# phoreproject/prysm

Measured on AMD Instinct MI355X. Metric: tree-hash leaves/sec @2^28 chunks (ssz.merkleHash, 32-B leaves), higher is better.
Workload: dtype u64 (Keccak lanes as u32 pairs)

## Files before the change

### prysm_amd/csrc/keccak_dev.hpp

```cpp
#pragma once
#include <hip/hip_runtime.h>
#include <stdint.h>

#include "plan_types.hpp"

namespace mk {

__constant__ uint32_t kRcLo[24] = {
    0x00000001u, 0x00008082u, 0x0000808Au, 0x80008000u, 0x0000808Bu, 0x80000001u,
    0x80008081u, 0x00008009u, 0x0000008Au, 0x00000088u, 0x80008009u, 0x8000000Au,
    0x8000808Bu, 0x0000008Bu, 0x00008089u, 0x00008003u, 0x00008002u, 0x00000080u,
    0x0000800Au, 0x8000000Au, 0x80008081u, 0x00008080u, 0x80000001u, 0x80008008u};
__constant__ uint32_t kRcHi[24] = {
    0x00000000u, 0x00000000u, 0x80000000u, 0x80000000u, 0x00000000u, 0x00000000u,
    0x80000000u, 0x80000000u, 0x00000000u, 0x00000000u, 0x00000000u, 0x00000000u,
    0x00000000u, 0x80000000u, 0x80000000u, 0x80000000u, 0x80000000u, 0x80000000u,
    0x00000000u, 0x80000000u, 0x80000000u, 0x80000000u, 0x00000000u, 0x80000000u};

__device__ __forceinline__ uint32_t xor3(uint32_t a, uint32_t b, uint32_t c) {
    return __builtin_amdgcn_bitop3_b32(a, b, c, 0x96);
}
__device__ __forceinline__ uint32_t chi3(uint32_t a, uint32_t b, uint32_t c) {
    return __builtin_amdgcn_bitop3_b32(a, b, c, 0xD2);
}
__device__ __forceinline__ uint32_t funnel(uint32_t hi, uint32_t lo, uint32_t s) {
    return __builtin_amdgcn_alignbit(hi, lo, s);
}

template <int N>
__device__ __forceinline__ void rotl64(uint32_t lo, uint32_t hi, uint32_t& olo, uint32_t& ohi) {
    if constexpr (N == 0) {
        olo = lo;
        ohi = hi;
    } else if constexpr (N == 32) {
        olo = hi;
        ohi = lo;
    } else if constexpr (N < 32) {
        ohi = funnel(hi, lo, 32 - N);
        olo = funnel(lo, hi, 32 - N);
    } else {
        ohi = funnel(lo, hi, 64 - N);
        olo = funnel(hi, lo, 64 - N);
    }
}

struct State {
    uint32_t lo[25];
    uint32_t hi[25];
};

__device__ __forceinline__ void zero(State& s) {
#pragma unroll
    for (int i = 0; i < 25; ++i) {
        s.lo[i] = 0u;
        s.hi[i] = 0u;
    }
}

#define MK_RHO(i)                                                                          \
    ((i) == 0 ? 0 : (i) == 1 ? 1 : (i) == 2 ? 62 : (i) == 3 ? 28 : (i) == 4 ? 27          \
   : (i) == 5 ? 36 : (i) == 6 ? 44 : (i) == 7 ? 6 : (i) == 8 ? 55 : (i) == 9 ? 20          \
   : (i) == 10 ? 3 : (i) == 11 ? 10 : (i) == 12 ? 43 : (i) == 13 ? 25 : (i) == 14 ? 39    \
   : (i) == 15 ? 41 : (i) == 16 ? 45 : (i) == 17 ? 15 : (i) == 18 ? 21 : (i) == 19 ? 8    \
   : (i) == 20 ? 18 : (i) == 21 ? 2 : (i) == 22 ? 61 : (i) == 23 ? 56 : 14)

template <int I>
__device__ __forceinline__ void rho_pi_one(const State& a, uint32_t (&blo)[25], uint32_t (&bhi)[25]) {
    constexpr int x = I % 5, y = I / 5;
    constexpr int dst = y + 5 * ((2 * x + 3 * y) % 5);
    rotl64<MK_RHO(I)>(a.lo[I], a.hi[I], blo[dst], bhi[dst]);
}

template <int... Is>
__device__ __forceinline__ void rho_pi_all(const State& a, uint32_t (&blo)[25], uint32_t (&bhi)[25],
                                           std::integer_sequence<int, Is...>) {
    (rho_pi_one<Is>(a, blo, bhi), ...);
}

__device__ __forceinline__ uint32_t ax3(uint32_t a, uint32_t b, uint32_t c) {
    uint32_t r;
    asm volatile("v_bitop3_b32 %0, %1, %2, %3 bitop3:0x96" : "=v"(r) : "v"(a), "v"(b), "v"(c));
    return r;
}
__device__ __forceinline__ uint32_t achi(uint32_t a, uint32_t b, uint32_t c) {
    uint32_t r;
    asm volatile("v_bitop3_b32 %0, %1, %2, %3 bitop3:0xd2" : "=v"(r) : "v"(a), "v"(b), "v"(c));
    return r;
}
template <int S>
__device__ __forceinline__ uint32_t aalign(uint32_t hi, uint32_t lo) {
    uint32_t r;
    asm volatile("v_alignbit_b32 %0, %1, %2, %3" : "=v"(r) : "v"(hi), "v"(lo), "i"(S));
    return r;
}
__device__ __forceinline__ uint32_t axs(uint32_t a, uint32_t s) {
    uint32_t r;
    asm volatile("v_xor_b32 %0, %1, %2" : "=v"(r) : "s"(s), "v"(a));
    return r;
}
template <int N>
__device__ __forceinline__ void arot(uint32_t lo, uint32_t hi, uint32_t& olo, uint32_t& ohi) {
    if constexpr (N == 0) {
        olo = lo;
        ohi = hi;
    } else if constexpr (N < 32) {
        ohi = aalign<32 - N>(hi, lo);
        olo = aalign<32 - N>(lo, hi);
    } else {
        ohi = aalign<64 - N>(lo, hi);
        olo = aalign<64 - N>(hi, lo);
    }
}
template <int I>
__device__ __forceinline__ void arho(const State& a, uint32_t (&blo)[25], uint32_t (&bhi)[25]) {
    constexpr int x = I % 5, y = I / 5;
    constexpr int dst = y + 5 * ((2 * x + 3 * y) % 5);
    arot<MK_RHO(I)>(a.lo[I], a.hi[I], blo[dst], bhi[dst]);
}
template <int... Is>
__device__ __forceinline__ void arho_all(const State& a, uint32_t (&blo)[25], uint32_t (&bhi)[25],
                                         std::integer_sequence<int, Is...>) {
    (arho<Is>(a, blo, bhi), ...);
}

template <bool BAR = false>
__device__ __forceinline__ void round_asm(State& s, uint32_t rclo, uint32_t rchi) {
    uint32_t clo[5], chi_[5];
#pragma unroll
    for (int x = 0; x < 5; ++x) {
        clo[x] = ax3(s.lo[x], s.lo[x + 5], s.lo[x + 10]);
        chi_[x] = ax3(s.hi[x], s.hi[x + 5], s.hi[x + 10]);
    }
#pragma unroll
    for (int x = 0; x < 5; ++x) {
        clo[x] = ax3(clo[x], s.lo[x + 15], s.lo[x + 20]);
        chi_[x] = ax3(chi_[x], s.hi[x + 15], s.hi[x + 20]);
    }
    uint32_t rlo[5], rhi[5];
#pragma unroll
    for (int x = 0; x < 5; ++x) arot<1>(clo[x], chi_[x], rlo[x], rhi[x]);
    if constexpr (BAR && MK_LOCK_BARS >= 2) __builtin_amdgcn_s_barrier();
#pragma unroll
    for (int i = 0; i < 25; ++i) {
        const int x = i % 5;
        s.lo[i] = ax3(s.lo[i], clo[(x + 4) % 5], rlo[(x + 1) % 5]);
        s.hi[i] = ax3(s.hi[i], chi_[(x + 4) % 5], rhi[(x + 1) % 5]);
    }
    uint32_t blo[25], bhi[25];
    arho_all(s, blo, bhi, std::make_integer_sequence<int, 25>{});
    if constexpr (BAR) __builtin_amdgcn_s_barrier();
#pragma unroll
    for (int y = 0; y < 5; ++y) {
#pragma unroll
        for (int x = 0; x < 5; ++x) {
            const int i = x + 5 * y;
            const int i1 = (x + 1) % 5 + 5 * y, i2 = (x + 2) % 5 + 5 * y;
            s.lo[i] = achi(blo[i], blo[i1], blo[i2]);
            s.hi[i] = achi(bhi[i], bhi[i1], bhi[i2]);
        }
    }
    s.lo[0] = axs(s.lo[0], rclo);
    s.hi[0] = axs(s.hi[0], rchi);
}

__device__ __forceinline__ void round_fn(State& s, uint32_t rclo, uint32_t rchi) { round_asm(s, rclo, rchi); }

#ifndef MK_ROUND_UNROLL
#define MK_ROUND_UNROLL 2
#endif
constexpr int kRoundUnroll = MK_ROUND_UNROLL;

__device__ __forceinline__ void keccak_f(State& s) {
#pragma unroll kRoundUnroll
    for (int r = 0; r < 24; ++r) round_fn(s, kRcLo[r], kRcHi[r]);
}

template <int X>
__device__ __forceinline__ void diag_rho(const State& s, const uint32_t (&clo)[5], const uint32_t (&chi_)[5],
                                         const uint32_t (&rlo)[5], const uint32_t (&rhi)[5], uint32_t (&blo)[5],
                                         uint32_t (&bhi)[5]) {
    constexpr int i = 6 * X;
    const uint32_t alo = xor3(s.lo[i], clo[(X + 4) % 5], rlo[(X + 1) % 5]);
    const uint32_t ahi = xor3(s.hi[i], chi_[(X + 4) % 5], rhi[(X + 1) % 5]);
    rotl64<MK_RHO(i)>(alo, ahi, blo[X], bhi[X]);
}

__device__ __forceinline__ void last_round_digest(State& s, uint32_t rclo, uint32_t rchi) {
    uint32_t clo[5], chi_[5];
#pragma unroll
    for (int x = 0; x < 5; ++x) {
        clo[x] = xor3(xor3(s.lo[x], s.lo[x + 5], s.lo[x + 10]), s.lo[x + 15], s.lo[x + 20]);
        chi_[x] = xor3(xor3(s.hi[x], s.hi[x + 5], s.hi[x + 10]), s.hi[x + 15], s.hi[x + 20]);
    }
    uint32_t rlo[5], rhi[5];
#pragma unroll
    for (int x = 0; x < 5; ++x) rotl64<1>(clo[x], chi_[x], rlo[x], rhi[x]);
    uint32_t blo[5], bhi[5];
    diag_rho<0>(s, clo, chi_, rlo, rhi, blo, bhi);
    diag_rho<1>(s, clo, chi_, rlo, rhi, blo, bhi);
    diag_rho<2>(s, clo, chi_, rlo, rhi, blo, bhi);
    diag_rho<3>(s, clo, chi_, rlo, rhi, blo, bhi);
    diag_rho<4>(s, clo, chi_, rlo, rhi, blo, bhi);
#pragma unroll
    for (int x = 0; x < 4; ++x) {
        s.lo[x] = chi3(blo[x], blo[(x + 1) % 5], blo[(x + 2) % 5]);
        s.hi[x] = chi3(bhi[x], bhi[(x + 1) % 5], bhi[(x + 2) % 5]);
    }
    s.lo[0] ^= rclo;
    s.hi[0] ^= rchi;
}

__device__ __forceinline__ void keccak_f_digest(State& s) {
#pragma unroll kRoundUnroll
    for (int r = 0; r < 22; ++r) round_fn(s, kRcLo[r], kRcHi[r]);
    round_fn(s, kRcLo[22], kRcHi[22]);
    last_round_digest(s, kRcLo[23], kRcHi[23]);
    asm volatile("" : "+v"(s.lo[0]), "+v"(s.hi[0]), "+v"(s.lo[1]), "+v"(s.hi[1]), "+v"(s.lo[2]), "+v"(s.hi[2]),
                 "+v"(s.lo[3]), "+v"(s.hi[3]));
}

__device__ __forceinline__ void keccak_f_lock(State& s) {
#pragma unroll kRoundUnroll
    for (int r = 0; r < 24; ++r) round_asm<true>(s, kRcLo[r], kRcHi[r]);
}
template <int K, typename F>
__device__ __forceinline__ void keccak_f_lock_mid(State& s, F&& mid) {
    static_assert(K >= 0 && K <= 24, "mid point");
    if constexpr (K == 0) mid();
#pragma unroll kRoundUnroll
    for (int r = 0; r < K; ++r) round_asm<true>(s, kRcLo[r], kRcHi[r]);
    if constexpr (K > 0) mid();
#pragma unroll kRoundUnroll
    for (int r = K; r < 24; ++r) round_asm<true>(s, kRcLo[r], kRcHi[r]);
}
template <int K1, int K2, typename F1, typename F2>
__device__ __forceinline__ void keccak_f_lock_mid2(State& s, F1&& m1, F2&& m2) {
    static_assert(K1 > 0 && K1 < K2 && K2 < 24, "mid points");
#pragma unroll kRoundUnroll
    for (int r = 0; r < K1; ++r) round_asm<true>(s, kRcLo[r], kRcHi[r]);
    m1();
#pragma unroll kRoundUnroll
    for (int r = K1; r < K2; ++r) round_asm<true>(s, kRcLo[r], kRcHi[r]);
    m2();
#pragma unroll kRoundUnroll
    for (int r = K2; r < 24; ++r) round_asm<true>(s, kRcLo[r], kRcHi[r]);
}
template <int K1, int K2, int K3, typename F1, typename F2, typename F3>
__device__ __forceinline__ void keccak_f_lock_mid3(State& s, F1&& m1, F2&& m2, F3&& m3) {
    static_assert(K1 > 0 && K1 < K2 && K2 < K3 && K3 < 24, "mid points");
#pragma unroll kRoundUnroll
    for (int r = 0; r < K1; ++r) round_asm<true>(s, kRcLo[r], kRcHi[r]);
    m1();
#pragma unroll kRoundUnroll
    for (int r = K1; r < K2; ++r) round_asm<true>(s, kRcLo[r], kRcHi[r]);
    m2();
#pragma unroll kRoundUnroll
    for (int r = K2; r < K3; ++r) round_asm<true>(s, kRcLo[r], kRcHi[r]);
    m3();
#pragma unroll kRoundUnroll
    for (int r = K3; r < 24; ++r) round_asm<true>(s, kRcLo[r], kRcHi[r]);
}
template <int K = 0, typename F>
__device__ __forceinline__ void keccak_f_digest_lock(State& s, F&& mid) {
    static_assert(K >= 0 && K <= 22, "mid point");
    if constexpr (K == 0) mid();
#pragma unroll kRoundUnroll
    for (int r = 0; r < K; ++r) round_asm<true>(s, kRcLo[r], kRcHi[r]);
    if constexpr (K > 0) mid();
#pragma unroll kRoundUnroll
    for (int r = K; r < 22; ++r) round_asm<true>(s, kRcLo[r], kRcHi[r]);
    round_asm<true>(s, kRcLo[22], kRcHi[22]);
    last_round_digest(s, kRcLo[23], kRcHi[23]);
    asm volatile("" : "+v"(s.lo[0]), "+v"(s.hi[0]), "+v"(s.lo[1]), "+v"(s.hi[1]), "+v"(s.lo[2]), "+v"(s.hi[2]),
                 "+v"(s.lo[3]), "+v"(s.hi[3]));
}
template <int K1, int K2, int K3, typename F1, typename F2, typename F3>
__device__ __forceinline__ void keccak_f_digest_lock_mid3(State& s, F1&& m1, F2&& m2, F3&& m3) {
    static_assert(K1 > 0 && K1 < K2 && K2 < K3 && K3 <= 22, "mid points");
#pragma unroll kRoundUnroll
    for (int r = 0; r < K1; ++r) round_asm<true>(s, kRcLo[r], kRcHi[r]);
    m1();
#pragma unroll kRoundUnroll
    for (int r = K1; r < K2; ++r) round_asm<true>(s, kRcLo[r], kRcHi[r]);
    m2();
#pragma unroll kRoundUnroll
    for (int r = K2; r < K3; ++r) round_asm<true>(s, kRcLo[r], kRcHi[r]);
    m3();
#pragma unroll kRoundUnroll
    for (int r = K3; r < 22; ++r) round_asm<true>(s, kRcLo[r], kRcHi[r]);
    round_asm<true>(s, kRcLo[22], kRcHi[22]);
    last_round_digest(s, kRcLo[23], kRcHi[23]);
    asm volatile("" : "+v"(s.lo[0]), "+v"(s.hi[0]), "+v"(s.lo[1]), "+v"(s.hi[1]), "+v"(s.lo[2]), "+v"(s.hi[2]),
                 "+v"(s.lo[3]), "+v"(s.hi[3]));
}
__device__ __forceinline__ void keccak_f_digest_lock(State& s) {
#pragma unroll kRoundUnroll
    for (int r = 0; r < 22; ++r) round_asm<true>(s, kRcLo[r], kRcHi[r]);
    round_asm<true>(s, kRcLo[22], kRcHi[22]);
    last_round_digest(s, kRcLo[23], kRcHi[23]);
    asm volatile("" : "+v"(s.lo[0]), "+v"(s.hi[0]), "+v"(s.lo[1]), "+v"(s.hi[1]), "+v"(s.lo[2]), "+v"(s.hi[2]),
                 "+v"(s.lo[3]), "+v"(s.hi[3]));
}

__device__ __forceinline__ void xor_lane(State& s, int i, uint2 w) {
    s.lo[i] ^= w.x;
    s.hi[i] ^= w.y;
}

template <int POS>
__device__ __forceinline__ void pad_const(State& s) {
    constexpr int lane = POS / 8, sh = (POS % 8) * 8;
    if constexpr (sh < 32)
        s.lo[lane] ^= 1u << sh;
    else
        s.hi[lane] ^= 1u << (sh - 32);
    s.hi[16] ^= 0x80000000u;
}

typedef unsigned int u32x4_t __attribute__((ext_vector_type(4)));
typedef unsigned int u32x2_t __attribute__((ext_vector_type(2)));
__device__ __forceinline__ uint4 ld_stream(const uint4* p) { return *p; }
__device__ __forceinline__ uint2 ld_stream(const uint2* p) { return *p; }

__device__ __forceinline__ void digest(const State& s, uint4& d0, uint4& d1) {
    d0 = make_uint4(s.lo[0], s.hi[0], s.lo[1], s.hi[1]);
    d1 = make_uint4(s.lo[2], s.hi[2], s.lo[3], s.hi[3]);
}

}

namespace mk {
namespace pair {

__device__ __forceinline__ uint32_t partner(uint32_t v) {
    return (uint32_t)__builtin_amdgcn_mov_dpp((int)v, 0xB1 , 0xF, 0xF, false);
}

template <int N>
__device__ __forceinline__ uint32_t rot(uint32_t own, uint32_t par) {
    if constexpr (N == 0)
        return own;
    else if constexpr (N == 32)
        return par;
    else if constexpr (N < 32)
        return funnel(own, par, 32 - N);
    else
        return funnel(par, own, 64 - N);
}

struct Half {
    uint32_t v[25];
};

template <int I>
__device__ __forceinline__ void rho_pi_one(const Half& a, uint32_t (&b)[25]) {
    constexpr int x = I % 5, y = I / 5;
    constexpr int dst = y + 5 * ((2 * x + 3 * y) % 5);
    constexpr int r = MK_RHO(I);
    if constexpr (r == 0)
        b[dst] = a.v[I];
    else
        b[dst] = rot<r>(a.v[I], partner(a.v[I]));
}

template <int... Is>
__device__ __forceinline__ void rho_pi_all(const Half& a, uint32_t (&b)[25], std::integer_sequence<int, Is...>) {
    (rho_pi_one<Is>(a, b), ...);
}

__device__ __forceinline__ void round_fn(Half& s, uint32_t rc_own) {
    uint32_t c[5], r[5];
#pragma unroll
    for (int x = 0; x < 5; ++x) c[x] = xor3(xor3(s.v[x], s.v[x + 5], s.v[x + 10]), s.v[x + 15], s.v[x + 20]);
#pragma unroll
    for (int x = 0; x < 5; ++x) r[x] = rot<1>(c[x], partner(c[x]));
#pragma unroll
    for (int i = 0; i < 25; ++i) s.v[i] = xor3(s.v[i], c[(i % 5 + 4) % 5], r[(i % 5 + 1) % 5]);
    uint32_t b[25];
    rho_pi_all(s, b, std::make_integer_sequence<int, 25>{});
#pragma unroll
    for (int y = 0; y < 5; ++y)
#pragma unroll
        for (int x = 0; x < 5; ++x)
            s.v[x + 5 * y] = chi3(b[x + 5 * y], b[(x + 1) % 5 + 5 * y], b[(x + 2) % 5 + 5 * y]);
    s.v[0] ^= rc_own;
}

__device__ __forceinline__ void keccak_f(Half& s, bool odd) {
#pragma unroll kRoundUnroll
    for (int r = 0; r < 24; ++r) round_fn(s, odd ? kRcHi[r] : kRcLo[r]);
}

__device__ __forceinline__ void zero(Half& s) {
#pragma unroll
    for (int i = 0; i < 25; ++i) s.v[i] = 0u;
}

}
}

namespace mk {
namespace ilv {

__constant__ uint32_t kRcE[24] = {
    0x00000001u, 0x00000000u, 0x00000000u, 0x00000000u, 0x00000001u, 0x00000001u,
    0x00000001u, 0x00000001u, 0x00000000u, 0x00000000u, 0x00000001u, 0x00000000u,
    0x00000001u, 0x00000001u, 0x00000001u, 0x00000001u, 0x00000000u, 0x00000000u,
    0x00000000u, 0x00000000u, 0x00000001u, 0x00000000u, 0x00000001u, 0x00000000u};
__constant__ uint32_t kRcO[24] = {
    0x00000000u, 0x00000089u, 0x8000008bu, 0x80008080u, 0x0000008bu, 0x00008000u,
    0x80008088u, 0x80000082u, 0x0000000bu, 0x0000000au, 0x00008082u, 0x00008003u,
    0x0000808bu, 0x8000000bu, 0x8000008au, 0x80000081u, 0x80000081u, 0x80000008u,
    0x00000083u, 0x80008003u, 0x80008088u, 0x80000088u, 0x00008000u, 0x80008082u};

__device__ __forceinline__ uint32_t partner(uint32_t v) {
    return (uint32_t)__builtin_amdgcn_mov_dpp((int)v, 0xB1 , 0xF, 0xF, false);
}
__device__ __forceinline__ uint32_t rot32(uint32_t x, uint32_t sh ) {
    return __builtin_amdgcn_alignbit(x, x, sh);
}

struct Half {
    uint32_t v[25];
};

template <int R>
__device__ __forceinline__ uint32_t rot(uint32_t own, uint32_t p) {
    if constexpr (R == 0) {
        return own;
    } else if constexpr (R % 2 == 0) {
        return rot32(own, 32 - R / 2);
    } else {
        constexpr uint32_t m = (R - 1) / 2;
        return partner(rot32(own, (32 - m - p) & 31u));
    }
}

template <int I>
__device__ __forceinline__ void rho_pi_one(const Half& a, uint32_t (&b)[25], uint32_t p) {
    constexpr int x = I % 5, y = I / 5;
    constexpr int dst = y + 5 * ((2 * x + 3 * y) % 5);
    b[dst] = rot<MK_RHO(I)>(a.v[I], p);
}

template <int... Is>
__device__ __forceinline__ void rho_pi_all(const Half& a, uint32_t (&b)[25], uint32_t p,
                                           std::integer_sequence<int, Is...>) {
    (rho_pi_one<Is>(a, b, p), ...);
}

__device__ __forceinline__ void round_fn(Half& s, uint32_t rc_own, uint32_t p) {
// ... 185 lines not shown
```

### prysm_amd/csrc/merkle_kernels.hip

```cpp
#include <hip/hip_runtime.h>
#include <stdint.h>

#include "keccak_dev.hpp"
#include "list_branch.hpp"
#include "merkle_kernels.hpp"
#include "tree_compact.hpp"
#include "tree_copy.hpp"

namespace mk {

__device__ __noinline__ void sponge_generic(const uint8_t* __restrict__ p, uint64_t la, uint32_t lz,
                                            bool lenc, uint64_t nval, uint4& d0, uint4& d1) {
    const uint64_t len = la + lz + (lenc ? 32u : 0u);
    const uint64_t nb = len / 136 + 1;
    const bool aligned = (((uintptr_t)p) & 7u) == 0;
    State s;
    zero(s);
    for (uint64_t b = 0; b < nb; ++b) {
        const uint64_t base = b * 136;
#pragma unroll
        for (int w = 0; w < 17; ++w) {
            const uint64_t m0 = base + 8u * w;
            uint32_t lo = 0, hi = 0;
            if (aligned && m0 + 8 <= la) {
// ... 12 lines not shown
                        byte = e < 8 ? (uint32_t)((nval >> (8 * e)) & 0xFF) : 0u;
                    }
                    if (k < 4)
                        lo |= byte << (8 * k);
                    else
                        hi |= byte << (8 * (k - 4));
                }
            }
            if (m0 <= len && len < m0 + 8) {
                const uint32_t k = (uint32_t)(len - m0);
                if (k < 4)
                    lo ^= 1u << (8 * k);
                else
                    hi ^= 1u << (8 * (k - 4));
            }
            if (b == nb - 1 && w == 16) hi ^= 0x80000000u;
            s.lo[w] ^= lo;
            s.hi[w] ^= hi;
        }
        keccak_f(s);
    }
    digest(s, d0, d1);
}

__device__ __forceinline__ void hash_pair(uint4 l0, uint4 l1, uint4 r0, uint4 r1, bool padded,
                                          uint4& d0, uint4& d1) {
    State s;
    zero(s);
    xor_lane(s, 0, make_uint2(l0.x, l0.y));
    xor_lane(s, 1, make_uint2(l0.z, l0.w));
    xor_lane(s, 2, make_uint2(l1.x, l1.y));
    xor_lane(s, 3, make_uint2(l1.z, l1.w));
    if (!padded) {
        xor_lane(s, 4, make_uint2(r0.x, r0.y));
        xor_lane(s, 5, make_uint2(r0.z, r0.w));
        xor_lane(s, 6, make_uint2(r1.x, r1.y));
        xor_lane(s, 7, make_uint2(r1.z, r1.w));
    }
    if (padded) keccak_f(s);
    if (padded)
        s.lo[3] ^= 1u;
    else
        s.lo[8] ^= 1u;
    s.hi[16] ^= 0x80000000u;
    keccak_f_digest(s);
    digest(s, d0, d1);
}

__device__ __forceinline__ void hash_final(uint4 r0, uint4 r1, uint64_t n, uint4& d0, uint4& d1) {
    State s;
    zero(s);
    xor_lane(s, 0, make_uint2(r0.x, r0.y));
    xor_lane(s, 1, make_uint2(r0.z, r0.w));
    xor_lane(s, 2, make_uint2(r1.x, r1.y));
    xor_lane(s, 3, make_uint2(r1.z, r1.w));
    xor_lane(s, 4, make_uint2((uint32_t)n, (uint32_t)(n >> 32)));
    s.lo[8] ^= 1u;
    s.hi[16] ^= 0x80000000u;
    keccak_f_digest(s);
    digest(s, d0, d1);
}

#define MK_MIN_WAVES 1

__device__ __forceinline__ void hash_window256(const uint4* __restrict__ w, uint4& d0, uint4& d1) {
    State s;
    zero(s);
    uint4 v[16];
#pragma unroll
    for (int k = 0; k < 16; ++k) v[k] = ld_stream(w + k);
#pragma unroll
    for (int k = 0; k < 8; ++k) {
        s.lo[2 * k] ^= v[k].x;
        s.hi[2 * k] ^= v[k].y;
        s.lo[2 * k + 1] ^= v[k].z;
        s.hi[2 * k + 1] ^= v[k].w;
    }
    s.lo[16] ^= v[8].x;
    s.hi[16] ^= v[8].y;
    keccak_f(s);
    s.lo[0] ^= v[8].z;
    s.hi[0] ^= v[8].w;
#pragma unroll
    for (int k = 0; k < 7; ++k) {
        s.lo[1 + 2 * k] ^= v[9 + k].x;
        s.hi[1 + 2 * k] ^= v[9 + k].y;
        s.lo[2 + 2 * k] ^= v[9 + k].z;
        s.hi[2 + 2 * k] ^= v[9 + k].w;
    }
    s.lo[15] ^= 1u;
    s.hi[16] ^= 0x80000000u;
    keccak_f_digest(s);
    digest(s, d0, d1);
}

#define MK_LEAF_SPLIT_WAVES 5
__device__ __forceinline__ void hash_window256_split(const uint4* __restrict__ w, uint4& d0, uint4& d1) {
    State s;
    uint4 v[9];
#pragma unroll
    for (int k = 0; k < 9; ++k) v[k] = ld_stream(w + k);
#pragma unroll
    for (int k = 0; k < 8; ++k) {
        s.lo[2 * k] = v[k].x;
        s.hi[2 * k] = v[k].y;
        s.lo[2 * k + 1] = v[k].z;
        s.hi[2 * k + 1] = v[k].w;
    }
    s.lo[16] = v[8].x;
    s.hi[16] = v[8].y;
    const uint32_t t0 = v[8].z, t1 = v[8].w;
#pragma unroll
    for (int k = 17; k < 25; ++k) s.lo[k] = s.hi[k] = 0;
    keccak_f(s);
    asm volatile("" ::: "memory");
    s.lo[0] ^= t0;
    s.hi[0] ^= t1;
    {
        uint4 u[4];
#pragma unroll
        for (int k = 0; k < 4; ++k) u[k] = ld_stream(w + 9 + k);
#pragma unroll
        for (int k = 0; k < 4; ++k) {
            s.lo[1 + 2 * k] ^= u[k].x;
            s.hi[1 + 2 * k] ^= u[k].y;
            s.lo[2 + 2 * k] ^= u[k].z;
            s.hi[2 + 2 * k] ^= u[k].w;
        }
    }
    {
        uint4 u[3];
#pragma unroll
        for (int k = 0; k < 3; ++k) u[k] = ld_stream(w + 13 + k);
#pragma unroll
        for (int k = 0; k < 3; ++k) {
            s.lo[9 + 2 * k] ^= u[k].x;
            s.hi[9 + 2 * k] ^= u[k].y;
            s.lo[10 + 2 * k] ^= u[k].z;
            s.hi[10 + 2 * k] ^= u[k].w;
        }
    }
    s.lo[15] ^= 1u;
    s.hi[16] ^= 0x80000000u;
    keccak_f_digest(s);
    digest(s, d0, d1);
}

__device__ __forceinline__ void hash_node_lock(uint4 l0, uint4 l1, uint4 r0, uint4 r1, uint4& d0, uint4& d1) {
    State s;
    s.lo[0] = l0.x; s.hi[0] = l0.y; s.lo[1] = l0.z; s.hi[1] = l0.w;
    s.lo[2] = l1.x; s.hi[2] = l1.y; s.lo[3] = l1.z; s.hi[3] = l1.w;
    s.lo[4] = r0.x; s.hi[4] = r0.y; s.lo[5] = r0.z; s.hi[5] = r0.w;
    s.lo[6] = r1.x; s.hi[6] = r1.y; s.lo[7] = r1.z; s.hi[7] = r1.w;
#pragma unroll
    for (int k = 8; k < 25; ++k) s.lo[k] = s.hi[k] = 0;
    s.lo[8] = 1u;
    s.hi[16] = 0x80000000u;
    keccak_f_digest_lock(s);
    digest(s, d0, d1);
}

__device__ __forceinline__ uint4 ld_node(const uint4* p) { return ld_stream(p); }

template <bool LEAF>
__device__ __forceinline__ void first_level_generic(const ReduceArgs& a, uint64_t j, uint4& d0, uint4& d1) {
    if constexpr (LEAF) {
        if (j < a.c1_full) {
            hash_window256(reinterpret_cast<const uint4*>(a.items) + j * 16, d0, d1);
            return;
        }
        const uint64_t lo = j * 2 * a.cb;
        uint64_t la;
        uint32_t lz;
        if (2 * j + 1 < a.nchunks) {
            la = (lo + 2 * a.cb < a.total ? lo + 2 * a.cb : a.total) - lo;
            lz = 0;
        } else {
            la = a.total - lo;
            lz = 128;
        }
        sponge_generic(a.items + lo, la, lz, false, 0, d0, d1);
    } else {
        const uint4* in = reinterpret_cast<const uint4*>(a.items);
        const uint4 l0 = in[4 * j], l1 = in[4 * j + 1];
        if (a.cin == 1 && !a.pad_at_one) {
            d0 = l0;
            d1 = l1;
            return;
        }
        const bool padded = !(2 * j + 1 < a.cin);
        uint4 r0 = make_uint4(0, 0, 0, 0), r1 = r0;
        if (!padded) {
            r0 = in[4 * j + 2];
            r1 = in[4 * j + 3];
        }
        hash_pair(l0, l1, r0, r1, padded, d0, d1);
    }
}

template <int NI>
__device__ __forceinline__ void reduce_levels_out(const ReduceArgs& a, uint4* lds, uint32_t tid, uint64_t lo1,
                                                  uint64_t c2, uint64_t m2, bool pair) {
    uint64_t c = c2, m = m2;
    int left = a.finalize ? 64 : (int)a.levels - (pair ? 2 : 1);
    int done = 0;
    while (left > 0 && (c > 1 || a.pad_at_one)) {
        const uint64_t mn = (m + 1) / 2;
        const bool act = tid < mn;
        uint4 l0, l1, r0 = make_uint4(0, 0, 0, 0), r1 = r0;
        bool padded = false;
        if (act) {
            l0 = lds[4 * tid];
            l1 = lds[4 * tid + 1];
            padded = !(2 * (uint64_t)tid + 1 < m);
            if (!padded) {
                r0 = lds[4 * tid + 2];
                r1 = lds[4 * tid + 3];
            }
        }
        __syncthreads();
        if (act) {
            uint4 d0, d1;
            hash_pair(l0, l1, r0, r1, padded, d0, d1);
            lds[2 * tid] = d0;
            lds[2 * tid + 1] = d1;
        }
        __syncthreads();
        c = (c + 1) / 2;
        m = mn;
        --left;
        ++done;
    }

    uint4* out = reinterpret_cast<uint4*>(a.out);
    if (a.finalize) {
        if (tid == 0) {
            uint4 d0, d1;
            hash_final(lds[0], lds[1], a.n_items, d0, d1);
            out[0] = d0;
            out[1] = d1;
        }
    } else {
        const uint64_t lo_out = (pair ? lo1 / 2 : lo1) >> done;
        for (uint32_t k = tid; k < m; k += kReduceThreads) {
            out[2 * (lo_out + k)] = lds[2 * k];
            out[2 * (lo_out + k) + 1] = lds[2 * k + 1];
        }
    }
}

template <bool LEAF, bool FAST, int NI>
__global__ __launch_bounds__(kReduceThreads, (LEAF && FAST) ? MK_LEAF_SPLIT_WAVES : MK_MIN_WAVES) void
k_reduce(ReduceArgs a) {
    constexpr uint64_t kSpan1 = 2 * NI * kReduceThreads;
    constexpr uint64_t kSpan2 = kSpan1 / 2;
    constexpr bool kSplit = LEAF && FAST;
    __shared__ uint4 lds[2 * kSpan2];
    const uint32_t tid = threadIdx.x;
    const uint64_t wg = a.wg_base + blockIdx.x;
    const uint64_t lo1 = wg * kSpan1;
    const uint64_t span1 = kSpan1;
    const uint64_t c1 = a.c1;
    const uint64_t m1 = (c1 - lo1) < span1 ? (c1 - lo1) : span1;
    const bool pair = a.levels >= 2 && (c1 > 1 || a.pad_at_one);
    const uint64_t c2 = pair ? (c1 + 1) / 2 : c1;
    const uint64_t m2 = pair ? (m1 + 1) / 2 : m1;

    if constexpr (kSplit) {
#pragma unroll 1
        for (int i = 0; i < NI; ++i) {
            const uint32_t q = i * kReduceThreads + tid;
            const uint4* w = reinterpret_cast<const uint4*>(a.items) + (lo1 + 2 * (uint64_t)q) * 16;
            uint4 l0, l1, r0, r1, d0, d1;
            hash_window256_split(w, d0, d1);
            lds[2 * q] = d0;
            lds[2 * q + 1] = d1;
            hash_window256_split(w + 16, r0, r1);
            l0 = lds[2 * q];
            l1 = lds[2 * q + 1];
            hash_pair(l0, l1, r0, r1, false, d0, d1);
            lds[2 * q] = d0;
            lds[2 * q + 1] = d1;
        }
    } else if constexpr (FAST) {
#pragma unroll 1
        for (int i = 0; i < NI; ++i) {
            const uint32_t q = i * kReduceThreads + tid;
            const uint64_t j0 = lo1 + 2 * (uint64_t)q;
            uint4 l0, l1, r0, r1, d0, d1;
            const uint4* in = reinterpret_cast<const uint4*>(a.items) + j0 * 4;
            hash_pair(ld_node(in), ld_node(in + 1), ld_node(in + 2), ld_node(in + 3), false, l0, l1);
            hash_pair(ld_node(in + 4), ld_node(in + 5), ld_node(in + 6), ld_node(in + 7), false, r0, r1);
            hash_pair(l0, l1, r0, r1, false, d0, d1);
            lds[2 * q] = d0;
            lds[2 * q + 1] = d1;
        }
    } else if (pair) {
#pragma unroll 1
        for (int i = 0; i < NI; ++i) {
            const uint32_t q = i * kReduceThreads + tid;
            if (q < m2) {
                const uint64_t j0 = lo1 + 2 * (uint64_t)q;
                uint4 l0, l1, r0 = make_uint4(0, 0, 0, 0), r1 = r0, d0, d1;
                first_level_generic<LEAF>(a, j0, l0, l1);
                const bool padded = !(2 * (uint64_t)q + 1 < m1);
                if (!padded) first_level_generic<LEAF>(a, j0 + 1, r0, r1);
                hash_pair(l0, l1, r0, r1, padded, d0, d1);
                lds[2 * q] = d0;
                lds[2 * q + 1] = d1;
            }
        }
    } else {
#pragma unroll 1
        for (int i = 0; i < NI; ++i) {
            const uint32_t q = i * kReduceThreads + tid;
            if (q < m1) {
                uint4 d0, d1;
                first_level_generic<LEAF>(a, lo1 + q, d0, d1);
                lds[2 * q] = d0;
                lds[2 * q + 1] = d1;
            }
        }
    }
    __syncthreads();

    reduce_levels_out<NI>(a, lds, tid, lo1, c2, m2, pair);
}

#define MK_LOCK_SPLIT_B1 4
#define MK_LOCK_SPLIT_B2 8
#define MK_LOCK_SPLIT_A1 2
#define MK_LOCK_SPLIT_A2 8
constexpr int kLockAux = 2;
constexpr int kSideAux = 0;
template <int NU, int U0, int AUX = 0, int I0 = 0, int I1 = NU>
__device__ __forceinline__ void lock_dma_c(uint4* Bw, const uint4* __restrict__ Rj, uint32_t lane) {
    asm volatile("" : "+v"(lane));
#pragma unroll
    for (int i = I0; i < I1; ++i) {
        const uint32_t U = 64u * i + lane;
        const uint32_t m = U / NU, u = U - m * NU;
        __builtin_amdgcn_global_load_lds(reinterpret_cast<const void*>(Rj + m * 64 + U0 + u),
                                         (__attribute__((address_space(3))) void*)(Bw + 64 * i), 16, 0, AUX);
    }
}
template <int I0 = 0, int I1 = 9>
__device__ __forceinline__ void lock_dma_a(uint4* Bw, const uint4* __restrict__ Rj, uint32_t lane) {
    asm volatile("" : "+v"(lane));
#pragma unroll
    for (int i = I0; i < I1; ++i) {
        const uint32_t U = 64u * i + lane;
        const uint32_t m = U / 9, u = U - m * 9;
        __builtin_amdgcn_global_load_lds(reinterpret_cast<const void*>(Rj + m * 64 + (u < 8 ? u : 7)),
                                         (__attribute__((address_space(3))) void*)(Bw + 64 * i), 16, 0, kLockAux);
    }
    if constexpr (I1 == 9)
        __builtin_amdgcn_global_load_lds(reinterpret_cast<const void*>(Rj + lane * 64 + 8),
                                         (__attribute__((address_space(3))) void*)(Bw + 576), 16, 0, 0);
}

template <typename F>
__device__ __forceinline__ void hash_window_sc(uint4* Bw, uint32_t lane, const uint4* __restrict__ Rj,
                                               const uint4* __restrict__ Rnext, uint4& d0, uint4& d1,
                                               F&& after_wait) {
    State s;
    asm volatile("s_waitcnt vmcnt(0)" ::: "memory");
    after_wait();
#pragma unroll
    for (int k = 0; k < 8; ++k) {
        const uint4 v = Bw[9 * lane + k];
        s.lo[2 * k] = v.x;
        s.hi[2 * k] = v.y;
        s.lo[2 * k + 1] = v.z;
        s.hi[2 * k + 1] = v.w;
    }
    const uint4 v8 = Bw[576 + lane];
    s.lo[16] = v8.x;
    s.hi[16] = v8.y;
#pragma unroll
    for (int k = 17; k < 25; ++k) s.lo[k] = s.hi[k] = 0;
    asm volatile("s_waitcnt lgkmcnt(0)" ::: "memory");
    lock_dma_c<7, 9, kLockAux, 0, 3>(Bw, Rj, lane);
    keccak_f_lock_mid2<MK_LOCK_SPLIT_B1, MK_LOCK_SPLIT_B2>(
        s, [&] { lock_dma_c<7, 9, kLockAux, 3, 5>(Bw, Rj, lane); },
        [&] { lock_dma_c<7, 9, kLockAux, 5, 7>(Bw, Rj, lane); });
    s.lo[0] ^= v8.z;
    s.hi[0] ^= v8.w;
    asm volatile("s_waitcnt vmcnt(0)" ::: "memory");
#pragma unroll
    for (int k = 0; k < 7; ++k) {
        const uint4 u = Bw[7 * lane + k];
        s.lo[1 + 2 * k] ^= u.x;
        s.hi[1 + 2 * k] ^= u.y;
        s.lo[2 + 2 * k] ^= u.z;
        s.hi[2 + 2 * k] ^= u.w;
    }
    asm volatile("s_waitcnt lgkmcnt(0)" ::: "memory");
    s.lo[15] ^= 1u;
    s.hi[16] ^= 0x80000000u;
    keccak_f_digest_lock_mid3<MK_LOCK_SPLIT_A1, MK_LOCK_SPLIT_A2, MK_LOCK_DMA_ROUND>(
        s, [&] { if (Rnext) lock_dma_a<0, 3>(Bw, Rnext, lane); },
        [&] { if (Rnext) lock_dma_a<3, 6>(Bw, Rnext, lane); },
        [&] { if (Rnext) lock_dma_a<6, 9>(Bw, Rnext, lane); });
    digest(s, d0, d1);
}

#if MK_TOP_STAMPS
__device__ uint64_t g_leaf_stamps[2 * 1024];
#endif
__global__ __launch_bounds__(kLockThreads, 1) void k_leaf_lock_sc(ReduceArgs a, uint64_t ngroups) {
#if MK_TOP_STAMPS
    if (threadIdx.x == 0 && blockIdx.x < 1024) g_leaf_stamps[2 * blockIdx.x] = __builtin_amdgcn_s_memrealtime();
#endif
    __shared__ uint4 buf[kLockThreads / 64][10 * 64];
    const uint32_t lane = threadIdx.x & 63u, wave = threadIdx.x >> 6;
    uint4* Bw = buf[wave];
    const uint4* items = reinterpret_cast<const uint4*>(a.items);
    uint4* out = reinterpret_cast<uint4*>(a.out);
    auto region = [&](uint64_t g) { return items + (g * kLockThreads + 64 * wave) * 64; };
    uint64_t g = blockIdx.x;
    if (g < ngroups) lock_dma_a(Bw, region(g), lane);
    uint4 q0 = make_uint4(0, 0, 0, 0), q1 = q0;
    uint64_t qnode = 0;
    bool pend = false;
    auto flush = [&] {
        if (pend) {
            out[2 * qnode] = q0;
            out[2 * qnode + 1] = q1;
        }
    };
    auto none = [] {};
#pragma unroll 1
    for (; g < ngroups; g += gridDim.x) {
        const uint4* R = region(g);
        const uint64_t gn = g + gridDim.x;
        const uint4* Rn = gn < ngroups ? region(gn) : nullptr;
        uint4 l0, l1, r0, r1, p0, p1;
        hash_window_sc(Bw, lane, R, R + 16, l0, l1, flush);
        hash_window_sc(Bw, lane, R + 16, R + 32, r0, r1, none);
        hash_node_lock(l0, l1, r0, r1, p0, p1);
        hash_window_sc(Bw, lane, R + 32, R + 48, l0, l1, none);
        hash_window_sc(Bw, lane, R + 48, Rn, r0, r1, none);
        hash_node_lock(l0, l1, r0, r1, l0, l1);
        hash_node_lock(p0, p1, l0, l1, q0, q1);
        qnode = g * kLockThreads + threadIdx.x;
        pend = true;
    }
    flush();
#if MK_TOP_STAMPS
    __syncthreads();
    if (threadIdx.x == 0 && blockIdx.x < 1024) g_leaf_stamps[2 * blockIdx.x + 1] = __builtin_amdgcn_s_memrealtime();
#endif
}

template __global__ void k_reduce<true, true, 2>(ReduceArgs);
template __global__ void k_reduce<true, false, 2>(ReduceArgs);
template __global__ void k_reduce<false, true, 2>(ReduceArgs);
template __global__ void k_reduce<false, false, 2>(ReduceArgs);
template __global__ void k_reduce<true, true, 1>(ReduceArgs);
template __global__ void k_reduce<true, false, 1>(ReduceArgs);


__device__ __forceinline__ void elem32_digest(const uint4* __restrict__ e, uint32_t (&d)[8]) {
    asm volatile("" ::: "memory");
    const uint4 v0 = ld_stream(e), v1 = ld_stream(e + 1);
    State s;
    s.lo[0] = 32u;
    s.hi[0] = v0.x;
    s.lo[1] = v0.y;
    s.hi[1] = v0.z;
    s.lo[2] = v0.w;
    s.hi[2] = v1.x;
    s.lo[3] = v1.y;
    s.hi[3] = v1.z;
    s.lo[4] = v1.w;
    s.hi[4] = 1u;
#pragma unroll
    for (int k = 5; k < 25; ++k) s.lo[k] = s.hi[k] = 0;
    s.hi[16] = 0x80000000u;
    keccak_f_digest(s);
    d[0] = s.lo[0];
    d[1] = s.hi[0];
    d[2] = s.lo[1];
    d[3] = s.hi[1];
    d[4] = s.lo[2];
    d[5] = s.hi[2];
    d[6] = s.lo[3];
    d[7] = s.hi[3];
}

__device__ __noinline__ void sponge_prefix4(const uint8_t* __restrict__ A, uint32_t L, uint4& d0, uint4& d1);

__device__ __noinline__ void elem_digest_any(const uint8_t* __restrict__ p, uint32_t L, uint32_t (&d)[8]) {
    uint4 d0, d1;
    if ((((uintptr_t)p) & 3u) == 0) {
        sponge_prefix4(p, L, d0, d1);
    } else {
        const uint64_t len = (uint64_t)L + 4;
        const uint64_t nb = len / 136 + 1;
        State s;
        zero(s);
        for (uint64_t b = 0; b < nb; ++b) {
#pragma unroll 1
            for (int w = 0; w < 17; ++w) {
                uint32_t h[2] = {0u, 0u};
#pragma unroll 1
                for (int k = 0; k < 8; ++k) {
                    const uint64_t m = b * 136 + 8u * w + k;
                    uint32_t byte = 0;
                    if (m < 4)
                        byte = (L >> (8 * m)) & 0xFFu;
                    else if (m < len)
                        byte = p[m - 4];
                    else if (m == len)
                        byte = 1u;
                    h[k >> 2] |= byte << (8 * (k & 3));
                }
                if (b == nb - 1 && w == 16) h[1] ^= 0x80000000u;
                s.lo[w] ^= h[0];
                s.hi[w] ^= h[1];
            }
            keccak_f(s);
        }
        digest(s, d0, d1);
    }
    d[0] = d0.x, d[1] = d0.y, d[2] = d0.z, d[3] = d0.w;
    d[4] = d1.x, d[5] = d1.y, d[6] = d1.z, d[7] = d1.w;
}

__device__ __forceinline__ void elem_window32(const uint4* __restrict__ w, uint32_t* stg, uint4& o0, uint4& o1) {
#pragma unroll
    for (int e = 4; e < 8; ++e) {
        uint32_t d[8];
        elem32_digest(w + 2 * e, d);
#pragma unroll
        for (int k = 0; k < 8; ++k) stg[(8 * (e - 4) + k) * kReduceThreads] = d[k];
    }
    uint32_t m[32];
#pragma unroll
    for (int e = 0; e < 4; ++e) {
        uint32_t d[8];
        elem32_digest(w + 2 * e, d);
#pragma unroll
        for (int k = 0; k < 8; ++k) m[8 * e + k] = d[k];
    }
    State s;
#pragma unroll
    for (int k = 0; k < 16; ++k) {
        s.lo[k] = m[2 * k];
        s.hi[k] = m[2 * k + 1];
    }
    s.lo[16] = stg[0];
    s.hi[16] = stg[kReduceThreads];
#pragma unroll
    for (int k = 17; k < 25; ++k) s.lo[k] = s.hi[k] = 0;
    keccak_f(s);
#pragma unroll
    for (int q = 0; q < 30; ++q) {
        const uint32_t v = stg[(2 + q) * kReduceThreads];
        if (q & 1)
            s.hi[q >> 1] ^= v;
        else
            s.lo[q >> 1] ^= v;
    }
    s.lo[15] ^= 1u;
    s.hi[16] ^= 0x80000000u;
    keccak_f_digest(s);
    digest(s, o0, o1);
}

__device__ __noinline__ void elem_window_generic(const ReduceArgs& a, uint64_t j, uint4& o0, uint4& o1) {
    const uint64_t n = a.n_items;
    const uint32_t cnt = (uint32_t)((n - 8 * j) < 8 ? (n - 8 * j) : 8);
    const bool padded = !(2 * j + 1 < a.nchunks);
    const uint32_t L = a.elem_len;
    uint32_t m[64];
#pragma unroll
    for (int e = 0; e < 8; ++e) {
        uint32_t d[8] = {0, 0, 0, 0, 0, 0, 0, 0};
        if ((uint32_t)e < cnt) elem_digest_any(a.items + (8 * j + e) * (uint64_t)L, L, d);
#pragma unroll
        for (int k = 0; k < 8; ++k) m[8 * e + k] = d[k];
    }
    const uint32_t lm = 32 * cnt + (padded ? 128u : 0u);
    const uint32_t nb = lm / 136 + 1;
    State s;
    zero(s);
#pragma unroll
    for (int b = 0; b < 2; ++b) {
        if ((uint32_t)b >= nb) break;
#pragma unroll
        for (int w = 0; w < 34; ++w) {
            const int q = 34 * b + w;
            uint32_t v = q < 64 ? m[q] : 0u;
            if ((uint32_t)q * 4 == lm) v ^= 1u;
// ... 3575 lines not shown
```

Baseline: 30.52 billion.

## Specialize Keccak round 0 for sparse states and precompute DMA lane offsets

Adds specialized first Keccak rounds for two known-sparse input states: a 64-byte node message with fixed padding, and a 17-lane absorbed block with zero capacity lanes. Zero lanes and padding constants are folded into theta so the XORs on zeros disappear and the zero-initialisation stores go away. The lock-step DMA address computation is also reworked. It now uses a per-lane precomputed seed and constant lane masks with cndmask instead of per-iteration divides by 7 and 9, and the wave index is made scalar via readfirstlane. This trims ALU work on both the hash and address paths, in exchange for more template and inline-asm complexity and some risk of address mistakes.

```diff
diff --git a/prysm_amd/csrc/keccak_dev.hpp b/prysm_amd/csrc/keccak_dev.hpp
--- a/prysm_amd/csrc/keccak_dev.hpp
+++ b/prysm_amd/csrc/keccak_dev.hpp
@@ -2,6 +2,7 @@
 #include <hip/hip_runtime.h>
 #include <stdint.h>
 
+#include "keccak_sparse.hpp"
 #include "plan_types.hpp"
 
 namespace mk {
@@ -165,6 +166,45 @@
 
 __device__ __forceinline__ void round_fn(State& s, uint32_t rclo, uint32_t rchi) { round_asm(s, rclo, rchi); }
 
+__device__ __forceinline__ uint32_t ax2(uint32_t a, uint32_t b) {
+    uint32_t r;
+    asm volatile("v_xor_b32 %0, %1, %2" : "=v"(r) : "v"(a), "v"(b));
+    return r;
+}
+__device__ __forceinline__ uint32_t ax3s(uint32_t a, uint32_t b, uint32_t s) {
+    uint32_t r;
+    asm volatile("v_bitop3_b32 %0, %1, %2, %3 bitop3:0x96" : "=v"(r) : "v"(a), "v"(b), "s"(s));
+    return r;
+}
+template <bool BAR>
+struct AsmOps {
+    static __device__ __forceinline__ uint32_t x2(uint32_t a, uint32_t b) { return ax2(a, b); }
+    static __device__ __forceinline__ uint32_t x3(uint32_t a, uint32_t b, uint32_t c) { return ax3(a, b, c); }
+    static __device__ __forceinline__ uint32_t xk(uint32_t a, uint32_t k) { return axs(a, k); }
+    static __device__ __forceinline__ uint32_t x3k(uint32_t a, uint32_t b, uint32_t k) { return ax3s(a, b, k); }
+    static __device__ __forceinline__ uint32_t chi(uint32_t a, uint32_t b, uint32_t c) { return achi(a, b, c); }
+    template <int N>
+    static __device__ __forceinline__ void rot(uint32_t lo, uint32_t hi, uint32_t& olo, uint32_t& ohi) {
+        arot<N>(lo, hi, olo, ohi);
+    }
+    static __device__ __forceinline__ void bar_theta() {
+        if constexpr (BAR && MK_LOCK_BARS >= 2) __builtin_amdgcn_s_barrier();
+    }
+    static __device__ __forceinline__ void bar_chi() {
+        if constexpr (BAR) __builtin_amdgcn_s_barrier();
+    }
+};
+enum Start { kAnyState = 0, kNodeMsg = 1, kBlock17 = 2 };
+template <Start ST, bool BAR>
+__device__ __forceinline__ void round0(State& s) {
+    if constexpr (ST == kNodeMsg)
+        sparse::round0_node<AsmOps<BAR>>(s, kRcLo[0], kRcHi[0]);
+    else if constexpr (ST == kBlock17)
+        sparse::round0_block17<AsmOps<BAR>>(s, kRcLo[0], kRcHi[0]);
+    else
+        round_asm<BAR>(s, kRcLo[0], kRcHi[0]);
+}
+
 #ifndef MK_ROUND_UNROLL
 #define MK_ROUND_UNROLL 2
 #endif
@@ -233,11 +273,12 @@
 #pragma unroll kRoundUnroll
     for (int r = K; r < 24; ++r) round_asm<true>(s, kRcLo[r], kRcHi[r]);
 }
-template <int K1, int K2, typename F1, typename F2>
+template <int K1, int K2, Start ST = kAnyState, typename F1, typename F2>
 __device__ __forceinline__ void keccak_f_lock_mid2(State& s, F1&& m1, F2&& m2) {
     static_assert(K1 > 0 && K1 < K2 && K2 < 24, "mid points");
-#pragma unroll kRoundUnroll
-    for (int r = 0; r < K1; ++r) round_asm<true>(s, kRcLo[r], kRcHi[r]);
+    if constexpr (ST != kAnyState) round0<ST, true>(s);
+#pragma unroll kRoundUnroll
+    for (int r = ST != kAnyState ? 1 : 0; r < K1; ++r) round_asm<true>(s, kRcLo[r], kRcHi[r]);
     m1();
 #pragma unroll kRoundUnroll
     for (int r = K1; r < K2; ++r) round_asm<true>(s, kRcLo[r], kRcHi[r]);
@@ -293,10 +334,17 @@
     asm volatile("" : "+v"(s.lo[0]), "+v"(s.hi[0]), "+v"(s.lo[1]), "+v"(s.hi[1]), "+v"(s.lo[2]), "+v"(s.hi[2]),
                  "+v"(s.lo[3]), "+v"(s.hi[3]));
 }
+template <Start ST = kAnyState>
 __device__ __forceinline__ void keccak_f_digest_lock(State& s) {
-#pragma unroll kRoundUnroll
-    for (int r = 0; r < 22; ++r) round_asm<true>(s, kRcLo[r], kRcHi[r]);
-    round_asm<true>(s, kRcLo[22], kRcHi[22]);
+    if constexpr (ST != kAnyState) {
+        round0<ST, true>(s);
+#pragma unroll kRoundUnroll
+        for (int r = 1; r < 23; ++r) round_asm<true>(s, kRcLo[r], kRcHi[r]);
+    } else {
+#pragma unroll kRoundUnroll
+        for (int r = 0; r < 22; ++r) round_asm<true>(s, kRcLo[r], kRcHi[r]);
+        round_asm<true>(s, kRcLo[22], kRcHi[22]);
+    }
     last_round_digest(s, kRcLo[23], kRcHi[23]);
     asm volatile("" : "+v"(s.lo[0]), "+v"(s.hi[0]), "+v"(s.lo[1]), "+v"(s.hi[1]), "+v"(s.lo[2]), "+v"(s.hi[2]),
                  "+v"(s.lo[3]), "+v"(s.hi[3]));
diff --git a/prysm_amd/csrc/keccak_sparse.hpp b/prysm_amd/csrc/keccak_sparse.hpp
--- /dev/null
+++ b/prysm_amd/csrc/keccak_sparse.hpp
@@ -0,0 +1,122 @@
+#pragma once
+#include <stdint.h>
+
+#include <utility>
+
+#if defined(__HIPCC__)
+#define MK_SPARSE_FN __device__ __forceinline__
+#else
+#define MK_SPARSE_FN inline
+#endif
+
+namespace mk {
+namespace sparse {
+
+constexpr int rho(int i) {
+    constexpr int r[25] = {0, 1, 62, 28, 27, 36, 44, 6, 55, 20, 3, 10, 43, 25, 39, 41, 45, 15, 21, 8, 18, 2, 61, 56, 14};
+    return r[i];
+}
+
+template <class Ops, class S, int I>
+MK_SPARSE_FN void rho_pi_one(const S& a, uint32_t (&blo)[25], uint32_t (&bhi)[25]) {
+    constexpr int x = I % 5, y = I / 5;
+    constexpr int dst = y + 5 * ((2 * x + 3 * y) % 5);
+    Ops::template rot<rho(I)>(a.lo[I], a.hi[I], blo[dst], bhi[dst]);
+}
+template <class Ops, class S, int... Is>
+MK_SPARSE_FN void rho_pi_all(const S& a, uint32_t (&blo)[25], uint32_t (&bhi)[25], std::integer_sequence<int, Is...>) {
+    (rho_pi_one<Ops, S, Is>(a, blo, bhi), ...);
+}
+
+template <class Ops, class S>
+MK_SPARSE_FN void tail(S& s, uint32_t rclo, uint32_t rchi) {
+    uint32_t blo[25], bhi[25];
+    rho_pi_all<Ops>(s, blo, bhi, std::make_integer_sequence<int, 25>{});
+    Ops::bar_chi();
+#pragma unroll
+    for (int y = 0; y < 5; ++y) {
+#pragma unroll
+        for (int x = 0; x < 5; ++x) {
+            const int i = x + 5 * y;
+            const int i1 = (x + 1) % 5 + 5 * y, i2 = (x + 2) % 5 + 5 * y;
+            s.lo[i] = Ops::chi(blo[i], blo[i1], blo[i2]);
+            s.hi[i] = Ops::chi(bhi[i], bhi[i1], bhi[i2]);
+        }
+    }
+    s.lo[0] = Ops::xk(s.lo[0], rclo);
+    s.hi[0] = Ops::xk(s.hi[0], rchi);
+}
+
+template <class Ops>
+MK_SPARSE_FN void theta_d(const uint32_t (&clo)[5], const uint32_t (&chi_)[5], uint32_t (&dlo)[5], uint32_t (&dhi)[5]) {
+    uint32_t rlo[5], rhi[5];
+#pragma unroll
+    for (int x = 0; x < 5; ++x) Ops::template rot<1>(clo[x], chi_[x], rlo[x], rhi[x]);
+    Ops::bar_theta();
+#pragma unroll
+    for (int x = 0; x < 5; ++x) {
+        dlo[x] = Ops::x2(clo[(x + 4) % 5], rlo[(x + 1) % 5]);
+        dhi[x] = Ops::x2(chi_[(x + 4) % 5], rhi[(x + 1) % 5]);
+    }
+}
+
+template <class Ops, class S>
+MK_SPARSE_FN void round0_node(S& s, uint32_t rclo, uint32_t rchi) {
+    uint32_t clo[5], chi_[5];
+    clo[0] = Ops::x2(s.lo[0], s.lo[5]);
+    chi_[0] = Ops::x2(s.hi[0], s.hi[5]);
+    clo[1] = Ops::x2(s.lo[1], s.lo[6]);
+    chi_[1] = Ops::x3k(s.hi[1], s.hi[6], 0x80000000u);
+    clo[2] = Ops::x2(s.lo[2], s.lo[7]);
+    chi_[2] = Ops::x2(s.hi[2], s.hi[7]);
+    clo[3] = Ops::xk(s.lo[3], 1u);
+    chi_[3] = s.hi[3];
+    clo[4] = s.lo[4];
+    chi_[4] = s.hi[4];
+    uint32_t dlo[5], dhi[5];
+    theta_d<Ops>(clo, chi_, dlo, dhi);
+#pragma unroll
+    for (int i = 0; i < 8; ++i) {
+        s.lo[i] = Ops::x2(s.lo[i], dlo[i % 5]);
+        s.hi[i] = Ops::x2(s.hi[i], dhi[i % 5]);
+    }
+#pragma unroll
+    for (int i = 8; i < 25; ++i) {
+        s.lo[i] = dlo[i % 5];
+        s.hi[i] = dhi[i % 5];
+    }
+    s.lo[8] = Ops::xk(s.lo[8], 1u);
+    s.hi[16] = Ops::xk(s.hi[16], 0x80000000u);
+    tail<Ops>(s, rclo, rchi);
+}
+
+template <class Ops, class S>
+MK_SPARSE_FN void round0_block17(S& s, uint32_t rclo, uint32_t rchi) {
+    uint32_t clo[5], chi_[5];
+#pragma unroll
+    for (int x = 0; x < 5; ++x) {
+        clo[x] = Ops::x3(s.lo[x], s.lo[x + 5], s.lo[x + 10]);
+        chi_[x] = Ops::x3(s.hi[x], s.hi[x + 5], s.hi[x + 10]);
+    }
+#pragma unroll
+    for (int x = 0; x < 2; ++x) {
+        clo[x] = Ops::x2(clo[x], s.lo[x + 15]);
+        chi_[x] = Ops::x2(chi_[x], s.hi[x + 15]);
+    }
+    uint32_t dlo[5], dhi[5];
+    theta_d<Ops>(clo, chi_, dlo, dhi);
+#pragma unroll
+    for (int i = 0; i < 17; ++i) {
+        s.lo[i] = Ops::x2(s.lo[i], dlo[i % 5]);
+        s.hi[i] = Ops::x2(s.hi[i], dhi[i % 5]);
+    }
+#pragma unroll
+    for (int i = 17; i < 25; ++i) {
+        s.lo[i] = dlo[i % 5];
+        s.hi[i] = dhi[i % 5];
+    }
+    tail<Ops>(s, rclo, rchi);
+}
+
+}
+}
diff --git a/prysm_amd/csrc/merkle_kernels.hip b/prysm_amd/csrc/merkle_kernels.hip
--- a/prysm_amd/csrc/merkle_kernels.hip
+++ b/prysm_amd/csrc/merkle_kernels.hip
@@ -188,11 +188,7 @@
     s.lo[2] = l1.x; s.hi[2] = l1.y; s.lo[3] = l1.z; s.hi[3] = l1.w;
     s.lo[4] = r0.x; s.hi[4] = r0.y; s.lo[5] = r0.z; s.hi[5] = r0.w;
     s.lo[6] = r1.x; s.hi[6] = r1.y; s.lo[7] = r1.z; s.hi[7] = r1.w;
-#pragma unroll
-    for (int k = 8; k < 25; ++k) s.lo[k] = s.hi[k] = 0;
-    s.lo[8] = 1u;
-    s.hi[16] = 0x80000000u;
-    keccak_f_digest_lock(s);
+    keccak_f_digest_lock<kNodeMsg>(s);
     digest(s, d0, d1);
 }
 
@@ -369,34 +365,80 @@
 #define MK_LOCK_SPLIT_A2 8
 constexpr int kLockAux = 2;
 constexpr int kSideAux = 0;
+__device__ __forceinline__ uint32_t lock_dma_seed(uint32_t lane) {
+    const uint32_t m9 = lane / 9, u9 = lane - 9 * m9, m7 = lane / 7, u7 = lane - 7 * m7;
+    return (1024 * m9 + 16 * u9) | (1024 * m7 + 16 * u7) << 16;
+}
+template <int NU>
+constexpr uint64_t lock_lanes_wrapped(int i) {
+    uint64_t s = 0;
+    for (int l = 0; l < 64; ++l) s |= (uint64_t)(l % NU + i >= NU) << l;
+    return s;
+}
+template <int NU>
+constexpr uint64_t lock_lanes_last(int i) {
+    uint64_t s = 0;
+    for (int l = 0; l < 64; ++l) s |= (uint64_t)((l + 64 * i) % NU == NU - 1) << l;
+    return s;
+}
+__device__ __forceinline__ uint32_t lock_sel0(uint32_t b, uint64_t lanes) {
+    uint32_t r;
+    asm("v_cndmask_b32_e64 %0, 0, %1, %2" : "=v"(r) : "v"(b), "s"(lanes));
+    return r;
+}
+template <int A>
+__device__ __forceinline__ uint32_t lock_sel_else(uint32_t b, uint64_t lanes) {
+    uint32_t r;
+    asm("v_cndmask_b32_e64 %0, %1, %2, %3" : "=v"(r) : "n"(A), "v"(b), "s"(lanes));
+    return r;
+}
+__device__ __forceinline__ uint32_t lock_clear(uint32_t a, uint64_t lanes) {
+    uint32_t r;
+    asm("v_cndmask_b32_e64 %0, %1, 0, %2" : "=v"(r) : "v"(a), "s"(lanes));
+    return r;
+}
+template <int A>
+__device__ __forceinline__ uint32_t lock_clear_imm(uint64_t lanes) {
+    uint32_t r;
+    asm("v_cndmask_b32_e64 %0, %1, 0, %2" : "=v"(r) : "n"(A), "s"(lanes));
+    return r;
+}
+template <int AUX>
+__device__ __forceinline__ void lock_dma_issue(uint4* row, const uint4* base, uint32_t off) {
+    asm("" : "+s"(base));
+    __builtin_amdgcn_global_load_lds(reinterpret_cast<const void*>(reinterpret_cast<const char*>(base) + off),
+                                     (__attribute__((address_space(3))) void*)row, 16, 0, AUX);
+}
 template <int NU, int U0, int AUX = 0, int I0 = 0, int I1 = NU>
-__device__ __forceinline__ void lock_dma_c(uint4* Bw, const uint4* __restrict__ Rj, uint32_t lane) {
-    asm volatile("" : "+v"(lane));
+__device__ __forceinline__ void lock_dma_c(uint4* Bw, const uint4* __restrict__ Rj, uint32_t seed) {
+    static_assert(NU == 7 && 63 % NU == 0, "the seed's high half is the stride-7 image");
+    asm volatile("" : "+v"(seed));
+    const uint32_t off0 = seed >> 16;
 #pragma unroll
     for (int i = I0; i < I1; ++i) {
-        const uint32_t U = 64u * i + lane;
-        const uint32_t m = U / NU, u = U - m * NU;
-        __builtin_amdgcn_global_load_lds(reinterpret_cast<const void*>(Rj + m * 64 + U0 + u),
-                                         (__attribute__((address_space(3))) void*)(Bw + 64 * i), 16, 0, AUX);
+        const uint32_t off = i ? off0 + lock_sel0(1024u - 16u * NU, lock_lanes_wrapped<NU>(i)) : off0;
+        lock_dma_issue<AUX>(Bw + 64 * i, Rj + (63 / NU) * 64 * i + i + U0, off);
     }
 }
 template <int I0 = 0, int I1 = 9>
-__device__ __forceinline__ void lock_dma_a(uint4* Bw, const uint4* __restrict__ Rj, uint32_t lane) {
-    asm volatile("" : "+v"(lane));
+__device__ __forceinline__ void lock_dma_a(uint4* Bw, const uint4* __restrict__ Rj, uint32_t seed, uint32_t lane) {
+    asm volatile("" : "+v"(seed));
+    const uint32_t off0 = seed & 0xFFFFu;
 #pragma unroll
     for (int i = I0; i < I1; ++i) {
-        const uint32_t U = 64u * i + lane;
-        const uint32_t m = U / 9, u = U - m * 9;
-        __builtin_amdgcn_global_load_lds(reinterpret_cast<const void*>(Rj + m * 64 + (u < 8 ? u : 7)),
-                                         (__attribute__((address_space(3))) void*)(Bw + 64 * i), 16, 0, kLockAux);
-    }
-    if constexpr (I1 == 9)
-        __builtin_amdgcn_global_load_lds(reinterpret_cast<const void*>(Rj + lane * 64 + 8),
-                                         (__attribute__((address_space(3))) void*)(Bw + 576), 16, 0, 0);
+        const uint32_t d = i ? lock_clear(lock_sel_else<16>(1024u - 16u * 9 + 16u, lock_lanes_wrapped<9>(i)),
+                                          lock_lanes_last<9>(i))
+                             : lock_clear_imm<16>(lock_lanes_last<9>(i));
+        lock_dma_issue<kLockAux>(Bw + 64 * i, Rj + 7 * 64 * i + i - 1, off0 + d);
+    }
+    if constexpr (I1 == 9) {
+        asm volatile("" : "+v"(lane));
+        lock_dma_issue<0>(Bw + 576, Rj + 8, lane << 10);
+    }
 }
 
 template <typename F>
-__device__ __forceinline__ void hash_window_sc(uint4* Bw, uint32_t lane, const uint4* __restrict__ Rj,
+__device__ __forceinline__ void hash_window_sc(uint4* Bw, uint32_t lane, uint32_t seed, const uint4* __restrict__ Rj,
                                                const uint4* __restrict__ Rnext, uint4& d0, uint4& d1,
                                                F&& after_wait) {
     State s;
@@ -413,13 +455,11 @@
     const uint4 v8 = Bw[576 + lane];
     s.lo[16] = v8.x;
     s.hi[16] = v8.y;
-#pragma unroll
-    for (int k = 17; k < 25; ++k) s.lo[k] = s.hi[k] = 0;
     asm volatile("s_waitcnt lgkmcnt(0)" ::: "memory");
-    lock_dma_c<7, 9, kLockAux, 0, 3>(Bw, Rj, lane);
-    keccak_f_lock_mid2<MK_LOCK_SPLIT_B1, MK_LOCK_SPLIT_B2>(
-        s, [&] { lock_dma_c<7, 9, kLockAux, 3, 5>(Bw, Rj, lane); },
-        [&] { lock_dma_c<7, 9, kLockAux, 5, 7>(Bw, Rj, lane); });
+    lock_dma_c<7, 9, kLockAux, 0, 3>(Bw, Rj, seed);
+    keccak_f_lock_mid2<MK_LOCK_SPLIT_B1, MK_LOCK_SPLIT_B2, kBlock17>(
+        s, [&] { lock_dma_c<7, 9, kLockAux, 3, 5>(Bw, Rj, seed); },
+        [&] { lock_dma_c<7, 9, kLockAux, 5, 7>(Bw, Rj, seed); });
     s.lo[0] ^= v8.z;
     s.hi[0] ^= v8.w;
     asm volatile("s_waitcnt vmcnt(0)" ::: "memory");
@@ -435,9 +475,9 @@
     s.lo[15] ^= 1u;
     s.hi[16] ^= 0x80000000u;
     keccak_f_digest_lock_mid3<MK_LOCK_SPLIT_A1, MK_LOCK_SPLIT_A2, MK_LOCK_DMA_ROUND>(
-        s, [&] { if (Rnext) lock_dma_a<0, 3>(Bw, Rnext, lane); },
-        [&] { if (Rnext) lock_dma_a<3, 6>(Bw, Rnext, lane); },
-        [&] { if (Rnext) lock_dma_a<6, 9>(Bw, Rnext, lane); });
+        s, [&] { if (Rnext) lock_dma_a<0, 3>(Bw, Rnext, seed, lane); },
+        [&] { if (Rnext) lock_dma_a<3, 6>(Bw, Rnext, seed, lane); },
+        [&] { if (Rnext) lock_dma_a<6, 9>(Bw, Rnext, seed, lane); });
     digest(s, d0, d1);
 }
 
@@ -449,13 +489,15 @@
     if (threadIdx.x == 0 && blockIdx.x < 1024) g_leaf_stamps[2 * blockIdx.x] = __builtin_amdgcn_s_memrealtime();
 #endif
     __shared__ uint4 buf[kLockThreads / 64][10 * 64];
-    const uint32_t lane = threadIdx.x & 63u, wave = threadIdx.x >> 6;
+    const uint32_t lane = threadIdx.x & 63u;
+    const uint32_t wave = __builtin_amdgcn_readfirstlane(threadIdx.x >> 6);
+    const uint32_t seed = lock_dma_seed(lane);
     uint4* Bw = buf[wave];
     const uint4* items = reinterpret_cast<const uint4*>(a.items);
     uint4* out = reinterpret_cast<uint4*>(a.out);
     auto region = [&](uint64_t g) { return items + (g * kLockThreads + 64 * wave) * 64; };
     uint64_t g = blockIdx.x;
-    if (g < ngroups) lock_dma_a(Bw, region(g), lane);
+    if (g < ngroups) lock_dma_a(Bw, region(g), seed, lane);
     uint4 q0 = make_uint4(0, 0, 0, 0), q1 = q0;
     uint64_t qnode = 0;
     bool pend = false;
@@ -472,11 +514,11 @@
         const uint64_t gn = g + gridDim.x;
         const uint4* Rn = gn < ngroups ? region(gn) : nullptr;
         uint4 l0, l1, r0, r1, p0, p1;
-        hash_window_sc(Bw, lane, R, R + 16, l0, l1, flush);
-        hash_window_sc(Bw, lane, R + 16, R + 32, r0, r1, none);
+        hash_window_sc(Bw, lane, seed, R, R + 16, l0, l1, flush);
+        hash_window_sc(Bw, lane, seed, R + 16, R + 32, r0, r1, none);
         hash_node_lock(l0, l1, r0, r1, p0, p1);
-        hash_window_sc(Bw, lane, R + 32, R + 48, l0, l1, none);
-        hash_window_sc(Bw, lane, R + 48, Rn, r0, r1, none);
+        hash_window_sc(Bw, lane, seed, R + 32, R + 48, l0, l1, none);
+        hash_window_sc(Bw, lane, seed, R + 48, Rn, r0, r1, none);
         hash_node_lock(l0, l1, r0, r1, l0, l1);
         hash_node_lock(p0, p1, l0, l1, q0, q1);
         qnode = g * kLockThreads + threadIdx.x;
```

Result: faster. 31.04 billion, median of 6 (+1.7%).
